# pyannote/pyannote-audio

Measured on AMD Instinct MI355X. Metric: audio-hours/sec (real-time factor) for speaker-diarization-3.1 pipeline, higher is better.
Workload: dtype f32

## Files before the change

### pyannote-audio_amd/csrc/seg_lstm.hip

```cpp
#include "common.h"

namespace pa {

constexpr int GB = 128;
constexpr int GK = 32;
constexpr int GLD = GK + 4;

template <int ACT, int OUT_MODE>
__global__ __launch_bounds__(256) void k_gemm_tn(const float* __restrict__ A, int lda,
                                                  const float* __restrict__ W, int ldw,
                                                  const float* __restrict__ bias,
                                                  const float* __restrict__ Res,
                                                  float* __restrict__ C, long ldc, int M, int N, int K,
                                                  int nm, int nn, int inner, long sAo, long sAi, long sWo,
                                                  long sWi, long sCo, long sCi, int gHW, int gWo, int gH, int gW) {
  if (gridDim.y > 1) {
    const int zo = blockIdx.y / inner, zi = blockIdx.y % inner;
    A += zo * sAo + zi * sAi;
    W += zo * sWo + zi * sWi;
    C += zo * sCo + zi * sCi;
    if (Res != nullptr) Res += zo * sCo + zi * sCi;
  }
  __shared__ __attribute__((aligned(16))) float As[GB * GLD];
  __shared__ __attribute__((aligned(16))) float Ws[GB * GLD];
  int mt, nt;
  const int bid = blockIdx.x;
  if (nn == 8) {
    nt = (bid >> 3) & 7;
    mt = (bid & 7) + 8 * (bid >> 6);
  } else {
    nt = bid % nn;
    mt = bid / nn;
  }
  if (mt >= nm) return;
  const int m0 = mt * GB, n0 = nt * GB;
  const int tid = threadIdx.x, lane = tid & 63, wv = tid >> 6;
  const int wm = wv >> 1, wn = wv & 1;
  const int lr = tid >> 3, lc = (tid & 7) * 4;

  float4 ra[4], rw[4];
  const float* ap[4];
  const float* wp[4];
#pragma unroll
  for (int i = 0; i < 4; ++i) {
    const int ar = m0 + lr + 32 * i, wr = n0 + lr + 32 * i;
    long arow = ar;
    if (gHW > 0) {
      const int b = ar / gHW, rem = ar - b * gHW, y = rem / gWo, x = rem - y * gWo;
      arow = ((long)b * gH + 2 * y) * gW + 2 * x;
    }
    ap[i] = ar < M ? A + arow * lda + lc : nullptr;
    wp[i] = wr < N ? W + (long)wr * ldw + lc : nullptr;
  }
  auto gload = [&](int k0) {
#pragma unroll
    for (int i = 0; i < 4; ++i) {
      ra[i] = ap[i] != nullptr ? *reinterpret_cast<const float4*>(ap[i] + k0) : make_float4(0.f, 0.f, 0.f, 0.f);
      rw[i] = wp[i] != nullptr ? *reinterpret_cast<const float4*>(wp[i] + k0) : make_float4(0.f, 0.f, 0.f, 0.f);
    }
  };
  auto lstore = [&]() {
#pragma unroll
    for (int i = 0; i < 4; ++i) {
      *reinterpret_cast<float4*>(As + (lr + 32 * i) * GLD + lc) = ra[i];
      *reinterpret_cast<float4*>(Ws + (lr + 32 * i) * GLD + lc) = rw[i];
    }
  };

  f32x16 acc[2][2];
#pragma unroll
  for (int i = 0; i < 2; ++i)
#pragma unroll
    for (int j = 0; j < 2; ++j)
#pragma unroll
      for (int r = 0; r < 16; ++r) acc[i][j][r] = 0.f;

  const int fi = lane & 31, kh = lane >> 5;
  gload(0);
  for (int k0 = 0; k0 < K; k0 += GK) {
    __syncthreads();
    lstore();
    __syncthreads();
    if (k0 + GK < K) gload(k0 + GK);
#pragma unroll
    for (int r4 = 0; r4 < 4; ++r4) {
      float4 af[2], wf[2];
#pragma unroll
      for (int i = 0; i < 2; ++i) {
        af[i] = *reinterpret_cast<const float4*>(As + (64 * wm + 32 * i + fi) * GLD + kh * 16 + 4 * r4);
        wf[i] = *reinterpret_cast<const float4*>(Ws + (64 * wn + 32 * i + fi) * GLD + kh * 16 + 4 * r4);
      }
#pragma unroll
      for (int i = 0; i < 2; ++i)
#pragma unroll
        for (int j = 0; j < 2; ++j) {
          acc[i][j] = MFMA32(af[i].x, wf[j].x, acc[i][j]);
          acc[i][j] = MFMA32(af[i].y, wf[j].y, acc[i][j]);
          acc[i][j] = MFMA32(af[i].z, wf[j].z, acc[i][j]);
          acc[i][j] = MFMA32(af[i].w, wf[j].w, acc[i][j]);
        }
    }
  }

#pragma unroll
  for (int i = 0; i < 2; ++i)
#pragma unroll
    for (int j = 0; j < 2; ++j) {
      const int n = n0 + 64 * wn + 32 * j + fi;
      const float bv = (bias != nullptr && n < N) ? bias[n] : 0.f;
#pragma unroll
      for (int q = 0; q < 4; ++q) {
        const int m = m0 + 64 * wm + 32 * i + 8 * q + 4 * kh;
        float v[4];
#pragma unroll
        for (int e = 0; e < 4; ++e) {
          v[e] = acc[i][j][4 * q + e] + bv;
          if (OUT_MODE == 0 && Res != nullptr && n < N && m + e < M) v[e] += Res[(long)(m + e) * ldc + n];
          if (ACT == 1) v[e] = leaky_relu(v[e]);
          if (ACT == 2) v[e] = fmaxf(v[e], 0.f);
          if (ACT == 3) v[e] = gelu_erf(v[e]);
        }
        if (n < N) {
          if (OUT_MODE == 0) {
#pragma unroll
            for (int e = 0; e < 4; ++e)
              if (m + e < M) C[(long)(m + e) * ldc + n] = v[e];
          } else {
            if (m < M)
              *reinterpret_cast<float4*>(C + ((long)(m >> 4) * N + n) * 16 + (m & 15)) =
                  make_float4(v[0], v[1], v[2], v[3]);
          }
        }
      }
    }
}

constexpr int LSTM_HS = 162;

__device__ __forceinline__ float sigmoidf_(float x) {
  return __builtin_amdgcn_rcpf(1.0f + __builtin_amdgcn_exp2f(-1.4426950408889634f * x));
}
__device__ __forceinline__ float tanhf_(float x) {
  const float xc = fminf(fmaxf(x, -15.f), 15.f);
  return 2.0f * __builtin_amdgcn_rcpf(1.0f + __builtin_amdgcn_exp2f(-2.8853900817779268f * xc)) - 1.0f;
}

__global__ __launch_bounds__(256, 1) void k_lstm_rec(const float* __restrict__ xproj,
                                                      const float* __restrict__ whh_p,
                                                      float* __restrict__ out, int T) {
  __shared__ float hs[2 * 16 * LSTM_HS];
  const int tile = blockIdx.x, dir = blockIdx.y;
  const int tid = threadIdx.x, lane = tid & 63, w = tid >> 6;
  const int n = lane & 15, g = lane >> 4;

  float wr[8][32];
  {
    const float* wp = whh_p + (long)((dir * 4 + w) * 8 * 32) * 64 + lane;
#pragma unroll
    for (int q8 = 0; q8 < 8; ++q8)
#pragma unroll
      for (int kt = 0; kt < 32; ++kt) wr[q8][kt] = wp[(q8 * 32 + kt) * 64];
  }
  for (int i = tid; i < 2 * 16 * LSTM_HS; i += 256) hs[i] = 0.f;
  float c[2][4];
#pragma unroll
  for (int s = 0; s < 2; ++s)
#pragma unroll
    for (int r = 0; r < 4; ++r) c[s][r] = 0.f;
  __syncthreads();

  const float* xbase = xproj + ((long)tile * T * 1024 + dir * 512 + w * 128 + n) * 16 + 4 * g;
  float* obase = out + ((long)tile * T * 16 + 4 * g) * 256 + dir * 128 + 32 * w + n;

  f32x4 xin[8];
  {
    const int t = dir ? T - 1 : 0;
#pragma unroll
    for (int q8 = 0; q8 < 8; ++q8)
      xin[q8] = *reinterpret_cast<const f32x4*>(xbase + ((long)t * 1024 + q8 * 16) * 16);
  }
  int cur = 0;
#pragma unroll 1
  for (int step = 0; step < T; ++step) {
    const int t = dir ? T - 1 - step : step;
    f32x4 acc[8];
#pragma unroll
    for (int q8 = 0; q8 < 8; ++q8) acc[q8] = xin[q8];
    if (step + 1 < T) {
      const int tn = dir ? t - 1 : t + 1;
#pragma unroll
      for (int q8 = 0; q8 < 8; ++q8)
        xin[q8] = *reinterpret_cast<const f32x4*>(xbase + ((long)tn * 1024 + q8 * 16) * 16);
    }
    const float* hp = hs + (cur * 16 + n) * LSTM_HS + g * 33;
    float a[32];
#pragma unroll
    for (int kt = 0; kt < 32; ++kt) a[kt] = hp[kt];
#pragma unroll
    for (int kt = 0; kt < 32; ++kt)
#pragma unroll
      for (int q8 = 0; q8 < 8; ++q8) acc[q8] = MFMA16(a[kt], wr[q8][kt], acc[q8]);

    float* hn = hs + ((cur ^ 1) * 16 + 4 * g) * LSTM_HS + w * 33 + n;
    float* op = obase + (long)t * 16 * 256;
#pragma unroll
    for (int s = 0; s < 2; ++s)
#pragma unroll
      for (int r = 0; r < 4; ++r) {
        const float ig = sigmoidf_(acc[0 + s][r]);
        const float fg = sigmoidf_(acc[2 + s][r]);
        const float gg = tanhf_(acc[4 + s][r]);
        const float og = sigmoidf_(acc[6 + s][r]);
        const float cn = fg * c[s][r] + ig * gg;
        c[s][r] = cn;
        const float h = og * tanhf_(cn);
        hn[r * LSTM_HS + 16 * s] = h;
        op[r * 256 + 16 * s] = h;
      }
    __syncthreads();
    cur ^= 1;
  }
}

constexpr int LSTMG_MT = 2;
constexpr int LSTMG_MAXU = 8;

__global__ __launch_bounds__(256) void k_lstm_rec_gen(const float* __restrict__ xproj,
                                                      const float* __restrict__ whh_g,
                                                      float* __restrict__ out, int T, int H, int ntiles,
                                                      int ndir, int hstride) {
  extern __shared__ float hsg[];
  constexpr int MT = LSTMG_MT;
  const int tile0 = blockIdx.x * MT, dir = blockIdx.y;
  const int tid = threadIdx.x, lane = tid & 63, w = tid >> 6;
  const int n = lane & 15, g = lane >> 4;
  const int U = H >> 4, K4 = H >> 4;
  const long NG = (long)ndir * 4 * H;
  const int ldo = ndir * H;
  for (int i = tid; i < MT * 2 * 16 * hstride; i += 256) hsg[i] = 0.f;
  f32x4 c[LSTMG_MAXU][MT];
#pragma unroll
  for (int ui = 0; ui < LSTMG_MAXU; ++ui)
#pragma unroll
    for (int mt = 0; mt < MT; ++mt) c[ui][mt] = f32x4{0.f, 0.f, 0.f, 0.f};
  __syncthreads();
  int tl[MT];
  bool live[MT];
#pragma unroll
  for (int mt = 0; mt < MT; ++mt) {
    live[mt] = tile0 + mt < ntiles;
    tl[mt] = live[mt] ? tile0 + mt : ntiles - 1;
  }
  int cur = 0;
#pragma unroll 1
  for (int step = 0; step < T; ++step) {
    const int t = dir ? T - 1 - step : step;
#pragma unroll
    for (int ui = 0; ui < LSTMG_MAXU; ++ui) {
      const int u = w + 4 * ui;
      if (u >= U) break;
      f32x4 xin[MT][4], acc[MT][4];
#pragma unroll
      for (int mt = 0; mt < MT; ++mt)
#pragma unroll
        for (int q = 0; q < 4; ++q) {
          xin[mt][q] = *reinterpret_cast<const f32x4*>(
              xproj + (((long)tl[mt] * T + t) * NG + (long)dir * 4 * H + (4 * u + q) * 16 + n) * 16 + 4 * g);
          acc[mt][q] = f32x4{0.f, 0.f, 0.f, 0.f};
        }
      const f32x4* wp = reinterpret_cast<const f32x4*>(whh_g) + ((long)(dir * U + u) * 4 * K4) * 64 + lane;
      const float* hp0 = hsg + (cur * 16 + n) * hstride + g;
#pragma unroll 2
      for (int k4 = 0; k4 < K4; ++k4) {
        f32x4 b[4];
#pragma unroll
        for (int q = 0; q < 4; ++q) b[q] = wp[(long)(q * K4 + k4) * 64];
#pragma unroll
        for (int j = 0; j < 4; ++j) {
#pragma unroll
          for (int mt = 0; mt < MT; ++mt) {
            const float a = hp0[mt * 2 * 16 * hstride + 16 * k4 + 4 * j];
#pragma unroll
            for (int q = 0; q < 4; ++q) acc[mt][q] = MFMA16(a, b[q][j], acc[mt][q]);
          }
        }
      }
#pragma unroll
      for (int mt = 0; mt < MT; ++mt) {
        float* hn = hsg + ((mt * 2 + (cur ^ 1)) * 16 + 4 * g) * hstride + 16 * u + n;
        float* op = out + (((long)tl[mt] * T + t) * 16 + 4 * g) * ldo + dir * H + 16 * u + n;
#pragma unroll
        for (int r = 0; r < 4; ++r) {
          const float ig = sigmoidf_(acc[mt][0][r] + xin[mt][0][r]);
          const float fg = sigmoidf_(acc[mt][1][r] + xin[mt][1][r]);
          const float gg = tanhf_(acc[mt][2][r] + xin[mt][2][r]);
          const float og = sigmoidf_(acc[mt][3][r] + xin[mt][3][r]);
          const float cn = fg * c[ui][mt][r] + ig * gg;
          c[ui][mt][r] = cn;
          const float h = og * tanhf_(cn);
          hn[r * hstride] = h;
          if (live[mt]) op[(long)r * ldo] = h;
        }
      }
    }
    __syncthreads();
    cur ^= 1;
  }
}

constexpr int CLS_MAXC = 16;

__global__ __launch_bounds__(256) void k_classifier(const float* __restrict__ X, int ldx, int K, int M,
                                                     int T, int B, const float* __restrict__ cw,
                                                     const float* __restrict__ cb, int NC,
                                                     const unsigned char* __restrict__ mapping, int S,
                                                     float* __restrict__ logp,
                                                     unsigned char* __restrict__ ml) {
  extern __shared__ float wsh[];
  for (int i = threadIdx.x; i < NC * K; i += 256) wsh[i] = cw[i];
  for (int i = threadIdx.x; i < NC; i += 256) wsh[NC * K + i] = cb[i];
  __syncthreads();
  const long m = (long)blockIdx.x * 256 + threadIdx.x;
  if (m >= M) return;
  const int b16 = (int)(m & 15);
  const long tt = m >> 4;
  const int t = (int)(tt % T), tile = (int)(tt / T);
  const int b = tile * 16 + b16;
  if (b >= B) return;
  float z[CLS_MAXC];
#pragma unroll
  for (int cidx = 0; cidx < CLS_MAXC; ++cidx) z[cidx] = cidx < NC ? wsh[NC * K + cidx] : 0.f;
  const float* x = X + m * ldx;
  for (int k = 0; k < K; k += 4) {
    const float4 xv = *reinterpret_cast<const float4*>(x + k);
#pragma unroll
    for (int cidx = 0; cidx < CLS_MAXC; ++cidx)
      if (cidx < NC) {
        const float* wrow = wsh + cidx * K + k;
        z[cidx] = fmaf(xv.x, wrow[0], z[cidx]);
        z[cidx] = fmaf(xv.y, wrow[1], z[cidx]);
        z[cidx] = fmaf(xv.z, wrow[2], z[cidx]);
        z[cidx] = fmaf(xv.w, wrow[3], z[cidx]);
      }
  }
  const long o = (long)b * T + t;
  if (mapping == nullptr) {
    if (logp != nullptr)
      for (int cidx = 0; cidx < NC; ++cidx) logp[o * NC + cidx] = 1.f / (1.f + expf(-z[cidx]));
    return;
  }
  float mx = z[0];
  int am = 0;
#pragma unroll
  for (int cidx = 1; cidx < CLS_MAXC; ++cidx)
    if (cidx < NC && z[cidx] > mx) {
      mx = z[cidx];
      am = cidx;
    }
  float se = 0.f;
#pragma unroll
  for (int cidx = 0; cidx < CLS_MAXC; ++cidx)
    if (cidx < NC) se += expf(z[cidx] - mx);
  const float lse = mx + logf(se);
  if (logp != nullptr)
    for (int cidx = 0; cidx < NC; ++cidx) logp[o * NC + cidx] = z[cidx] - lse;
  if (ml != nullptr)
    for (int s = 0; s < S; ++s) ml[o * S + s] = mapping[am * S + s];
}

}

extern "C" {

int pa_gemm_tn_ex(const float* A, int lda, const float* W, int ldw, const float* bias, const float* Res,
                  float* C, long ldc, int M, int N, int K, int act, int out_mode, void* stream);

int pa_gemm_tn(const float* A, int lda, const float* W, int ldw, const float* bias, float* C, long ldc,
               int M, int N, int K, int act, int out_mode, void* stream) {
  return pa_gemm_tn_ex(A, lda, W, ldw, bias, nullptr, C, ldc, M, N, K, act, out_mode, stream);
}

int pa_gemm_tn_batched(const float* A, int lda, long sAo, long sAi, const float* W, int ldw, long sWo, long sWi,
                       const float* bias, float* C, long ldc, long sCo, long sCi, int M, int N, int K,
                       int outer, int inner, int act, void* stream);

static int gemm_tn_launch(const float* A, int lda, const float* W, int ldw, const float* bias, const float* Res,
                          float* C, long ldc, int M, int N, int K, int act, int out_mode, int gHW, int gWo, int gH,
                          int gW, void* stream);

int pa_gemm_tn_ex(const float* A, int lda, const float* W, int ldw, const float* bias, const float* Res,
                  float* C, long ldc, int M, int N, int K, int act, int out_mode, void* stream) {
  return gemm_tn_launch(A, lda, W, ldw, bias, Res, C, ldc, M, N, K, act, out_mode, 0, 0, 0, 0, stream);
}

int pa_gemm_tn_s2(const float* X, int B, int H, int W, int cin, const float* Wt, int ldw, const float* bias, float* C,
                  long ldc, int N, void* stream) {
  const int Ho = (H - 1) / 2 + 1, Wo = (W - 1) / 2 + 1;
  if (B <= 0) return 0;
  return gemm_tn_launch(X, cin, Wt, ldw, bias, nullptr, C, ldc, B * Ho * Wo, N, cin, 0, 0, Ho * Wo, Wo, H, W, stream);
}

static int gemm_tn_launch(const float* A, int lda, const float* W, int ldw, const float* bias, const float* Res,
                          float* C, long ldc, int M, int N, int K, int act, int out_mode, int gHW, int gWo, int gH,
                          int gW, void* stream) {
  if (M <= 0 || N <= 0) return 0;
  PA_REQUIRE(Res == nullptr || out_mode == 0, "pa_gemm_tn_ex: a residual needs out_mode 0");
  PA_REQUIRE(K % pa::GK == 0 && lda % 4 == 0 && ldw % 4 == 0,
             "pa_gemm_tn: K (%d) must be a multiple of 32 and lda/ldw multiples of 4", K);
  PA_REQUIRE(out_mode == 0 || (M % 16 == 0), "pa_gemm_tn: out_mode 1 needs M %% 16 == 0");
  const int nm = pa::cdiv(M, pa::GB), nn = pa::cdiv(N, pa::GB);
  const int grid = nn == 8 ? pa::cdiv(nm, 8) * 64 : nm * nn;
  hipStream_t st = (hipStream_t)stream;
  pa::ProfScope prof("k_gemm_tn", stream, 2.0 * M * N * K, 4.0 * ((double)M * K + (double)N * K + (double)M * N));
#define PA_GEMM(ACT, OM)                                                                          \
  hipLaunchKernelGGL((pa::k_gemm_tn<ACT, OM>), dim3(grid), dim3(256), 0, st, A, lda, W, ldw, bias, \
                     Res, C, ldc, M, N, K, nm, nn, 1, 0L, 0L, 0L, 0L, 0L, 0L, gHW, gWo, gH, gW)
  if (act == 0 && out_mode == 0) PA_GEMM(0, 0);
  else if (act == 1 && out_mode == 0) PA_GEMM(1, 0);
  else if (act == 2 && out_mode == 0) PA_GEMM(2, 0);
  else if (act == 3 && out_mode == 0) PA_GEMM(3, 0);
  else if (act == 0 && out_mode == 1) PA_GEMM(0, 1);
  else PA_REQUIRE(false, "pa_gemm_tn: unsupported act/out_mode %d/%d", act, out_mode);
#undef PA_GEMM
  PA_CHECK_LAUNCH("pa_gemm_tn");
  return 0;
}

int pa_gemm_tn_batched(const float* A, int lda, long sAo, long sAi, const float* W, int ldw, long sWo, long sWi,
                       const float* bias, float* C, long ldc, long sCo, long sCi, int M, int N, int K,
                       int outer, int inner, int act, void* stream) {
  if (M <= 0 || N <= 0 || outer <= 0 || inner <= 0) return 0;
  PA_REQUIRE(K % pa::GK == 0 && lda % 4 == 0 && ldw % 4 == 0 && sAo % 4 == 0 && sAi % 4 == 0 && sWo % 4 == 0 &&
                 sWi % 4 == 0,
             "pa_gemm_tn_batched: K (%d) must be a multiple of 32 and every stride a multiple of 4", K);
  PA_REQUIRE((long)outer * inner <= 65535, "pa_gemm_tn_batched: at most 65535 products per launch");
  const int nm = pa::cdiv(M, pa::GB), nn = pa::cdiv(N, pa::GB);
  const int grid = nn == 8 ? pa::cdiv(nm, 8) * 64 : nm * nn;
  hipStream_t st = (hipStream_t)stream;
  const double z = (double)outer * inner;
  pa::ProfScope prof("k_gemm_tn", stream, 2.0 * z * M * N * K, 4.0 * z * ((double)M * K + (double)N * K + (double)M * N));
#define PA_GEMMB(ACT)                                                                                          \
  hipLaunchKernelGGL((pa::k_gemm_tn<ACT, 0>), dim3(grid, outer * inner), dim3(256), 0, st, A, lda, W, ldw, bias, \
                     (const float*)nullptr, C, ldc, M, N, K, nm, nn, inner, sAo, sAi, sWo, sWi, sCo, sCi, 0, 0, 0, 0)
  if (act == 0) PA_GEMMB(0);
  else if (act == 3) PA_GEMMB(3);
  else PA_REQUIRE(false, "pa_gemm_tn_batched: unsupported act %d", act);
#undef PA_GEMMB
  PA_CHECK_LAUNCH("pa_gemm_tn_batched");
  return 0;
}

int pa_lstm_rec(const float* xproj, const float* whh_packed, float* out, int ntiles, int ndir, int T,
                void* stream) {
  if (ntiles <= 0 || T <= 0) return 0;
  pa::ProfScope prof("k_lstm_rec", stream, 2.0 * ntiles * 16 * ndir * T * 128 * 512,
                     4.0 * ntiles * 16 * ndir * T * (512 + 128));
  hipLaunchKernelGGL(pa::k_lstm_rec, dim3(ntiles, ndir), dim3(256), 0, (hipStream_t)stream, xproj,
                     whh_packed, out, T);
  PA_CHECK_LAUNCH("pa_lstm_rec");
  return 0;
}

int pa_lstm_rec_h(const float* xproj, const float* whh_packed, float* out, int ntiles, int ndir, int T, int H,
                  void* stream) {
  if (ntiles <= 0 || T <= 0) return 0;
  if (H == 128 && ndir == 2) return pa_lstm_rec(xproj, whh_packed, out, ntiles, ndir, T, stream);
  PA_REQUIRE(H >= 16 && H % 16 == 0 && H <= 64 * pa::LSTMG_MAXU && (ndir == 1 || ndir == 2),
             "pa_lstm_rec_h: hidden size %d must be a multiple of 16 in [16, %d], directions 1 or 2 (got %d)", H,
             64 * pa::LSTMG_MAXU, ndir);
  const int hstride = ((H + 63) / 64) * 64 + 4;
  const size_t lds = sizeof(float) * pa::LSTMG_MT * 2 * 16 * hstride;
  {
    int dev = 0, limit = 0;
    (void)hipGetDevice(&dev);
    (void)hipDeviceGetAttribute(&limit, hipDeviceAttributeMaxSharedMemoryPerBlock, dev);
    PA_REQUIRE(limit <= 0 || lds <= (size_t)limit,
               "pa_lstm_rec_h: hidden size %d needs %zu bytes of LDS per workgroup, this device offers %d", H, lds, limit);
    static size_t granted = 0;
    if (lds > granted) {
      PA_REQUIRE(hipFuncSetAttribute((const void*)pa::k_lstm_rec_gen, hipFuncAttributeMaxDynamicSharedMemorySize,
                                     (int)lds) == hipSuccess,
                 "pa_lstm_rec_h: cannot reserve %zu bytes of dynamic LDS for hidden size %d", lds, H);
      granted = lds;
    }
  }
  pa::ProfScope prof("k_lstm_rec_gen", stream, 2.0 * ntiles * 16 * ndir * T * H * 4.0 * H,
                     4.0 * ntiles * 16 * ndir * T * (4.0 * H + H));
  hipLaunchKernelGGL(pa::k_lstm_rec_gen, dim3(pa::cdiv(ntiles, pa::LSTMG_MT), ndir), dim3(256), lds,
                     (hipStream_t)stream, xproj, whh_packed, out, T, H, ntiles, ndir, hstride);
  PA_CHECK_LAUNCH("pa_lstm_rec_h");
  return 0;
}

int pa_classifier(const float* X, int ldx, int K, int ntiles, int T, int B, const float* cw,
                  const float* cb, int NC, const unsigned char* mapping, int S, float* logp,
                  unsigned char* multilabel, void* stream) {
  PA_REQUIRE(NC <= pa::CLS_MAXC && K % 4 == 0, "pa_classifier: NC <= 16 and K %% 4 == 0 required");
  const long M = (long)ntiles * T * 16;
  if (M <= 0) return 0;
  const size_t lds = (size_t)(NC * K + NC) * sizeof(float);
  pa::ProfScope prof("k_classifier", stream, 2.0 * M * K * NC, 4.0 * M * K + 4.0 * M * NC);
  hipLaunchKernelGGL(pa::k_classifier, dim3(pa::cdiv(M, 256)), dim3(256), lds, (hipStream_t)stream, X,
                     ldx, K, (int)M, T, B, cw, cb, NC, mapping, S, logp, multilabel);
  PA_CHECK_LAUNCH("pa_classifier");
  return 0;
}

}
```

Measured before the change: 1.344.

## Prefetch LSTM input projections into LDS and add opt-in persistent gate GEMM

The LSTM recurrence kernel gains a variant, on by default, that prefetches the next timestep's input projection through buffer_load-to-LDS instructions interleaved with the MFMA chain. It then reads that data from LDS after the gate math, instead of holding the next step's inputs in VGPRs via global loads. This aims to hide global latency on the serial recurrent critical path, at the cost of 64KB of dynamic LDS. A new persistent, tile-queue-driven gate GEMM kernel with direct-to-LDS loads and a blocked output layout is also added, but it is only used when PA_GATE_GEMM is set.

```diff
diff --git a/pyannote-audio_amd/csrc/seg_gemm_gates.hip b/pyannote-audio_amd/csrc/seg_gemm_gates.hip
--- /dev/null
+++ b/pyannote-audio_amd/csrc/seg_gemm_gates.hip
@@ -0,0 +1,310 @@
+#include "common.h"
+
+namespace pa {
+
+constexpr int GG_B = 128;
+constexpr int GG_K = 32;
+constexpr int GG_IMG = GG_B * GG_K * 4;
+constexpr int GG_W_BASE = 2 * GG_IMG;
+constexpr int GG_BIAS_BASE = 4 * GG_IMG;
+constexpr int GG_MAIL = GG_BIAS_BASE + 2048;
+constexpr int GG_LDS = GG_MAIL + 16;
+constexpr int GG_OOB = (int)0x80000000;
+constexpr int GG_PIECES = 8;
+constexpr int GG_TILE_STORES = 16;
+#define GG_STR2(x) #x
+#define GG_STR(x) GG_STR2(x)
+#define GG_TAIL_WAIT_LIT 16
+static_assert(GG_TILE_STORES == GG_TAIL_WAIT_LIT, "the literal of the s_waitcnt string");
+
+typedef __attribute__((address_space(3))) unsigned char* gg_lds_t;
+typedef const volatile f32x4 __attribute__((address_space(3))) * gg_lds_f32x4_ptr;
+typedef const volatile float __attribute__((address_space(3))) * gg_lds_f32_ptr;
+__device__ __forceinline__ f32x4 gg_lds_read128(gg_lds_t p) { return *(gg_lds_f32x4_ptr)p; }
+
+__device__ __forceinline__ void gg_barrier() {
+  asm volatile("s_waitcnt lgkmcnt(0)" ::: "memory");
+  __builtin_amdgcn_s_barrier();
+  asm volatile("" ::: "memory");
+}
+
+template <int IMM>
+__device__ __forceinline__ void gg_piece(unsigned dst, int voff, __amdgpu_buffer_rsrc_t srd, int soff) {
+  asm volatile("s_add_u32 m0, %0, %1\n\ts_nop 0\n\tbuffer_load_dwordx4 %2, %3, %4 offen lds"
+               :: "s"(dst), "i"(IMM), "v"(voff), "s"(srd), "s"(soff)
+               : "memory", "scc");
+}
+struct GgStage {
+  __amdgpu_buffer_rsrc_t asrd, wsrd, bsrd;
+  int soff;
+  unsigned adst, wdst;
+  unsigned bdst;
+  bool with_bias;
+};
+template <int N>
+__device__ __forceinline__ void gg_issue(const GgStage& st, const int (&aoff)[4], const int (&woff)[4]) {
+  if constexpr (N < 4) gg_piece<4096 * N>(st.adst, aoff[N], st.asrd, st.soff);
+  else gg_piece<4096 * (N - 4)>(st.wdst, woff[N - 4], st.wsrd, st.soff);
+}
+__device__ __forceinline__ void gg_issue_n(const int n, const GgStage& st, const int (&aoff)[4], const int (&woff)[4]) {
+  switch (n) {
+#define GG_CASE(I) case I: gg_issue<I>(st, aoff, woff); break;
+    GG_CASE(0) GG_CASE(1) GG_CASE(2) GG_CASE(3) GG_CASE(4) GG_CASE(5) GG_CASE(6) GG_CASE(7)
+#undef GG_CASE
+    default: break;
+  }
+}
+
+__global__ __launch_bounds__(256, 2) void k_gemm_gates(const float* __restrict__ A, int lda,
+                                                       const float* __restrict__ W, int ldw,
+                                                       const float* __restrict__ bias, float* __restrict__ C, int M,
+                                                       int N, int K, int nm, int nn, int* __restrict__ counters) {
+  extern __shared__ __attribute__((aligned(16))) unsigned char smem_gg[];
+  const gg_lds_t lds = (gg_lds_t)smem_gg;
+  const unsigned lds0 = (unsigned)(size_t)lds;
+  int* mail = reinterpret_cast<int*>(smem_gg + GG_MAIL);
+
+  const int tid = threadIdx.x, lane = tid & 63;
+  const int slw = __builtin_amdgcn_readfirstlane(tid >> 6);
+  const int wm = slw >> 1, wn = slw & 1;
+  const int fi = lane & 31, kh = lane >> 5;
+
+  struct Tile {
+    int m0, n0;
+  };
+  auto mt_of = [&](int t) { return ((t >> 3) / nn) * 8 + (t & 7); };
+  auto decode = [&](int t) {
+    Tile q;
+    q.m0 = mt_of(t) * GG_B;
+    q.n0 = ((t >> 3) % nn) * GG_B;
+    return q;
+  };
+  auto resolve = [&](const TileQueue& tqq, int r) {
+    for (;;) {
+      const int t = tq_resolve(tqq, r);
+      if (t < 0 || mt_of(t) < nm) return t;
+      r = tq_claim_own(tqq);
+    }
+  };
+
+  gg_lds_t pa_[4], pw_[4];
+#pragma unroll
+  for (int r4 = 0; r4 < 4; ++r4) {
+    const int slot = ((4 * kh + r4) ^ ((fi >> 1) & 7)) * 16;
+    pa_[r4] = lds + (64 * wm + fi) * 128 + slot;
+    pw_[r4] = lds + GG_W_BASE + (64 * wn + fi) * 128 + slot;
+    asm volatile("" : "+v"(pa_[r4]));
+    asm volatile("" : "+v"(pw_[r4]));
+  }
+  const int drow = 8 * slw + (lane >> 3);
+  const int dslot = (lane & 7) ^ (4 * (slw & 1) + (lane >> 4));
+  int woff[4], aoff[4], arel[4];
+#pragma unroll
+  for (int j = 0; j < 4; ++j) {
+    woff[j] = ((drow + 32 * j) * ldw + 4 * dslot) * 4;
+    arel[j] = ((drow + 32 * j) * lda + 4 * dslot) * 4;
+  }
+  auto tile_offsets = [&](const Tile& q) {
+    const int rows = M - q.m0;
+#pragma unroll
+    for (int j = 0; j < 4; ++j) aoff[j] = drow + 32 * j < rows ? arel[j] : GG_OOB;
+  };
+  const int boff = lane < 32 ? lane * 16 : GG_OOB;
+  auto a_srd = [&](const Tile& q, bool live) {
+    const int rows = M - q.m0 < GG_B ? M - q.m0 : GG_B;
+    return __builtin_amdgcn_make_buffer_rsrc(const_cast<float*>(A + (long)q.m0 * lda), 0,
+                                             live ? ((rows - 1) * lda + K) * 4 : 0, 0x00020000);
+  };
+  auto w_srd = [&](const Tile& q, bool live) {
+    return __builtin_amdgcn_make_buffer_rsrc(const_cast<float*>(W + (long)q.n0 * ldw), 0,
+                                             live ? ((GG_B - 1) * ldw + K) * 4 : 0, 0x00020000);
+  };
+  auto b_srd = [&](const Tile& q, bool live) {
+    return __builtin_amdgcn_make_buffer_rsrc(const_cast<float*>(bias != nullptr ? bias + q.n0 : W), 0,
+                                             bias != nullptr && live ? GG_B * 4 : 0, 0x00020000);
+  };
+
+  const int per_xcd = ((nm + 7) >> 3) * nn;
+  const TileQueue tq{counters, (int)(blockIdx.x & 7), per_xcd};
+  if (tid == 0) mail[0] = resolve(tq, tq_claim_own(tq));
+  __syncthreads();
+  const int t0 = __builtin_amdgcn_readfirstlane(mail[0]);
+  if (t0 < 0) {
+    if (tid == 0) tq_done(tq, gridDim.x);
+    return;
+  }
+  Tile cur = decode(t0), nxt = cur;
+  __amdgpu_buffer_rsrc_t acur = a_srd(cur, true), wcur = w_srd(cur, true);
+  tile_offsets(cur);
+  {
+    GgStage st;
+    st.asrd = acur;
+    st.wsrd = wcur;
+    st.soff = 0;
+    st.adst = lds0 + 1024 * slw;
+    st.wdst = lds0 + GG_W_BASE + 1024 * slw;
+#pragma unroll
+    for (int n = 0; n < GG_PIECES; ++n) gg_issue_n(n, st, aoff, woff);
+    if (slw == 0) gg_piece<0>(lds0 + GG_BIAS_BASE, boff, b_srd(cur, true), 0);
+  }
+  int claim = 0;
+  if (tid == 0) claim = tq_claim_own(tq);
+  const int nst = K / GG_K;
+  int buf = 0, par = 0, tn = -1;
+  bool first_tile = true;
+
+  for (;;) {
+    f32x16 acc[2][2];
+#pragma unroll
+    for (int i = 0; i < 2; ++i)
+#pragma unroll
+      for (int j = 0; j < 2; ++j)
+#pragma unroll
+        for (int r = 0; r < 16; ++r) acc[i][j][r] = 0.f;
+    for (int s = 0; s < nst; ++s) {
+      const bool last = s == nst - 1;
+      if (s == 0 && !first_tile) asm volatile("s_waitcnt vmcnt(" GG_STR(GG_TAIL_WAIT_LIT) ")" ::: "memory");
+      else asm volatile("s_waitcnt vmcnt(0)" ::: "memory");
+      if (last && tid == 0) mail[par ^ 1] = resolve(tq, claim);
+      gg_barrier();
+      GgStage st;
+      auto setup = [&]() {
+        st.asrd = acur;
+        st.wsrd = wcur;
+        st.bsrd = wcur;
+        if (last) {
+          tn = __builtin_amdgcn_readfirstlane(mail[par ^ 1]);
+          if (tn >= 0) {
+            nxt = decode(tn);
+            tile_offsets(nxt);
+          }
+          st.asrd = a_srd(nxt, tn >= 0);
+          st.wsrd = w_srd(nxt, tn >= 0);
+          st.bsrd = b_srd(nxt, tn >= 0);
+        }
+        st.soff = last ? 0 : (s + 1) * GG_K * 4;
+        st.adst = lds0 + (buf ^ 1) * GG_IMG + 1024 * slw;
+        st.wdst = lds0 + GG_W_BASE + (buf ^ 1) * GG_IMG + 1024 * slw;
+        st.bdst = lds0 + GG_BIAS_BASE + (par ^ 1) * 1024;
+        st.with_bias = last && slw == 0;
+      };
+
+      {
+        f32x4 fa[2][2], fw[2][2];
+        auto rd = [&](const int r4, const int n, const int p) {
+          if (n == 0) fa[p][0] = gg_lds_read128(pa_[r4]);
+          else if (n == 1) fw[p][0] = gg_lds_read128(pw_[r4]);
+          else if (n == 2) fw[p][1] = gg_lds_read128(pw_[r4] + 4096);
+          else fa[p][1] = gg_lds_read128(pa_[r4] + 4096);
+        };
+#pragma unroll
+        for (int n = 0; n < 4; ++n) rd(0, n, 0);
+        __builtin_amdgcn_sched_barrier(0);
+        setup();
+        __builtin_amdgcn_sched_barrier(0);
+#pragma unroll
+        for (int r4 = 0; r4 < 4; ++r4) {
+          const int p = r4 & 1;
+#pragma unroll
+          for (int m = 0; m < 16; ++m) {
+            const int e = m >> 2, i = (m >> 1) & 1, j = m & 1;
+            acc[i][j] = MFMA32(fa[p][i][e], fw[p][j][e], acc[i][j]);
+            __builtin_amdgcn_sched_barrier(0);
+            if (r4 + 1 < 4 && m < 4) {
+              rd(r4 + 1, m, p ^ 1);
+              __builtin_amdgcn_sched_barrier(0);
+            }
+            const int idx = 16 * r4 + m;
+            if ((idx & 7) == 5) {
+              gg_issue_n(idx >> 3, st, aoff, woff);
+              __builtin_amdgcn_sched_barrier(0);
+            }
+            if (idx == 62) {
+              if (st.with_bias) gg_piece<0>(st.bdst, boff, st.bsrd, 0);
+              __builtin_amdgcn_sched_barrier(0);
+            }
+          }
+        }
+      }
+      {
+        const int d = buf ? -GG_IMG : GG_IMG;
+#pragma unroll
+        for (int r4 = 0; r4 < 4; ++r4) {
+          pa_[r4] += d;
+          pw_[r4] += d;
+          asm volatile("" : "+v"(pa_[r4]));
+          asm volatile("" : "+v"(pw_[r4]));
+        }
+      }
+      buf ^= 1;
+    }
+    if (tid == 0 && tn >= 0) claim = tq_claim_own(tq);
+    first_tile = false;
+    {
+      const int gv = (M - cur.m0) >> 4;
+      const __amdgpu_buffer_rsrc_t csrd = __builtin_amdgcn_make_buffer_rsrc(
+          C + ((long)(cur.m0 >> 4) * N + cur.n0) * 16, 0, (((gv < 8 ? gv : 8) - 1) * N + GG_B) * 64, 0x00020000);
+      const gg_lds_f32_ptr bl = (gg_lds_f32_ptr)(lds + GG_BIAS_BASE + par * 1024 + (64 * wn + fi) * 4);
+      const float bv[2] = {bl[0], bl[32]};
+      const int lane_base = (64 * wn + (fi & 15)) * 64 + (fi >> 4) * 32 + kh * 16;
+#pragma unroll
+      for (int i = 0; i < 2; ++i)
+#pragma unroll
+        for (int gg = 0; gg < 2; ++gg) {
+          const int gl = 4 * wm + 2 * i + gg;
+          const int voff = gl < gv ? gl * N * 64 + lane_base : GG_OOB;
+#pragma unroll
+          for (int j = 0; j < 2; ++j) {
+            u32x4 x, y;
+#pragma unroll
+            for (int e = 0; e < 4; ++e) {
+              const float lo = acc[i][j][8 * gg + e] + bv[j], hi = acc[i][j][8 * gg + 4 + e] + bv[j];
+              const auto r = __builtin_amdgcn_permlane16_swap(__builtin_bit_cast(unsigned int, lo),
+                                                              __builtin_bit_cast(unsigned int, hi), false, false);
+              x[e] = r[0];
+              y[e] = r[1];
+            }
+            __builtin_amdgcn_raw_buffer_store_b128(x, csrd, voff + j * 2048, 0, 0);
+            __builtin_amdgcn_raw_buffer_store_b128(y, csrd, voff + (j * 2048 + 1024), 0, 0);
+            asm volatile("s_nop 1" ::: "memory");
+            __builtin_amdgcn_sched_barrier(0);
+          }
+        }
+    }
+    if (tn < 0) break;
+    cur = nxt;
+    acur = a_srd(cur, true);
+    wcur = w_srd(cur, true);
+    par ^= 1;
+  }
+  if (tid == 0) tq_done(tq, gridDim.x);
+}
+
+int launch_gemm_gates(const float* A, int lda, const float* W, int ldw, const float* bias, float* C, int M, int N,
+                      int K, hipStream_t st) {
+  constexpr int MAXDEV = 16;
+  static int resident_of[MAXDEV] = {0};
+  int dev = 0;
+  (void)hipGetDevice(&dev);
+  if (dev < 0 || dev >= MAXDEV) dev = 0;
+  if (!resident_of[dev]) {
+    (void)hipFuncSetAttribute((const void*)k_gemm_gates, hipFuncAttributeMaxDynamicSharedMemorySize, GG_LDS);
+    int cus = 256;
+    (void)hipDeviceGetAttribute(&cus, hipDeviceAttributeMultiprocessorCount, dev);
+    resident_of[dev] = 2 * cus;
+  }
+  const int resident = resident_of[dev] & ~7;
+  const int nm = cdiv(M, GG_B), nn = N / GG_B;
+  const long total = (long)nm * nn;
+  const int grid = (int)(total < resident ? total : resident);
+  int* counters = tile_counters();
+  if (counters == nullptr) {
+    set_error("pa_gemm_tn: cannot allocate the tile counters");
+    return 2;
+  }
+  hipLaunchKernelGGL(k_gemm_gates, dim3(grid), dim3(256), GG_LDS, st, A, lda, W, ldw, bias, C, M, N, K, nm, nn,
+                     counters);
+  return 0;
+}
+
+}
diff --git a/pyannote-audio_amd/csrc/seg_lstm.hip b/pyannote-audio_amd/csrc/seg_lstm.hip
--- a/pyannote-audio_amd/csrc/seg_lstm.hip
+++ b/pyannote-audio_amd/csrc/seg_lstm.hip
@@ -145,10 +145,22 @@
   return 2.0f * __builtin_amdgcn_rcpf(1.0f + __builtin_amdgcn_exp2f(-2.8853900817779268f * xc)) - 1.0f;
 }
 
+constexpr int LSTM_XIN_WAVE = 2 * 8 * 1024;
+typedef __attribute__((address_space(3))) unsigned char* lstm_lds_t;
+typedef const volatile f32x4 __attribute__((address_space(3))) * lstm_lds_f32x4_ptr;
+template <int IMM>
+__device__ __forceinline__ void lstm_xin_piece(unsigned dst, int voff, __amdgpu_buffer_rsrc_t srd, int soff) {
+  asm volatile("s_add_u32 m0, %0, %1\n\ts_nop 0\n\tbuffer_load_dwordx4 %2, %3, %4 offen lds"
+               :: "s"(dst), "i"(IMM), "v"(voff), "s"(srd), "s"(soff)
+               : "memory", "scc");
+}
+
+template <bool XLDS>
 __global__ __launch_bounds__(256, 1) void k_lstm_rec(const float* __restrict__ xproj,
                                                       const float* __restrict__ whh_p,
                                                       float* __restrict__ out, int T) {
   __shared__ float hs[2 * 16 * LSTM_HS];
+  extern __shared__ __attribute__((aligned(16))) unsigned char xin_lds[];
   const int tile = blockIdx.x, dir = blockIdx.y;
   const int tid = threadIdx.x, lane = tid & 63, w = tid >> 6;
   const int n = lane & 15, g = lane >> 4;
@@ -172,12 +184,37 @@
   const float* xbase = xproj + ((long)tile * T * 1024 + dir * 512 + w * 128 + n) * 16 + 4 * g;
   float* obase = out + ((long)tile * T * 16 + 4 * g) * 256 + dir * 128 + 32 * w + n;
 
+  const int slw = __builtin_amdgcn_readfirstlane(w);
+  const __amdgpu_buffer_rsrc_t xsrd = __builtin_amdgcn_make_buffer_rsrc(
+      const_cast<float*>(xproj + ((long)tile * T * 1024 + dir * 512 + slw * 128) * 16), 0,
+      XLDS ? (T - 1) * 65536 + 8192 : 0, 0x00020000);
+  const int xvoff = n * 64 + g * 16;
+  const unsigned xdst = (unsigned)(size_t)(lstm_lds_t)xin_lds + slw * LSTM_XIN_WAVE;
+  lstm_lds_t xrd = (lstm_lds_t)xin_lds + slw * LSTM_XIN_WAVE + lane * 16;
+  auto xin_piece = [&](const int P, unsigned dst, __amdgpu_buffer_rsrc_t srd, int soff) {
+    switch (P) {
+#define PA_XIN_CASE(I) case I: lstm_xin_piece<I * 1024>(dst, xvoff, srd, soff + I * 1024); break;
+      PA_XIN_CASE(0) PA_XIN_CASE(1) PA_XIN_CASE(2) PA_XIN_CASE(3) PA_XIN_CASE(4) PA_XIN_CASE(5) PA_XIN_CASE(6)
+      PA_XIN_CASE(7)
+#undef PA_XIN_CASE
+      default: break;
+    }
+  };
+
   f32x4 xin[8];
   {
     const int t = dir ? T - 1 : 0;
-#pragma unroll
-    for (int q8 = 0; q8 < 8; ++q8)
-      xin[q8] = *reinterpret_cast<const f32x4*>(xbase + ((long)t * 1024 + q8 * 16) * 16);
+    if constexpr (XLDS) {
+#pragma unroll
+      for (int P = 0; P < 8; ++P) xin_piece(P, xdst, xsrd, t * 65536);
+      asm volatile("s_waitcnt vmcnt(0)" ::: "memory");
+#pragma unroll
+      for (int q8 = 0; q8 < 8; ++q8) xin[q8] = *(lstm_lds_f32x4_ptr)(xrd + q8 * 1024);
+    } else {
+#pragma unroll
+      for (int q8 = 0; q8 < 8; ++q8)
+        xin[q8] = *reinterpret_cast<const f32x4*>(xbase + ((long)t * 1024 + q8 * 16) * 16);
+    }
   }
   int cur = 0;
 #pragma unroll 1
@@ -186,11 +223,19 @@
     f32x4 acc[8];
 #pragma unroll
     for (int q8 = 0; q8 < 8; ++q8) acc[q8] = xin[q8];
-    if (step + 1 < T) {
-      const int tn = dir ? t - 1 : t + 1;
-#pragma unroll
-      for (int q8 = 0; q8 < 8; ++q8)
-        xin[q8] = *reinterpret_cast<const f32x4*>(xbase + ((long)tn * 1024 + q8 * 16) * 16);
+    const bool more = step + 1 < T;
+    const __amdgpu_buffer_rsrc_t nsrd = __builtin_amdgcn_make_buffer_rsrc(
+        const_cast<float*>(xproj + ((long)tile * T * 1024 + dir * 512 + slw * 128) * 16), 0,
+        XLDS && more ? (T - 1) * 65536 + 8192 : 0, 0x00020000);
+    const unsigned ndst = xdst + (cur ^ 1) * 8192;
+    const int nsoff = more ? (dir ? t - 1 : t + 1) * 65536 : 0;
+    if constexpr (!XLDS) {
+      if (step + 1 < T) {
+        const int tn = dir ? t - 1 : t + 1;
+#pragma unroll
+        for (int q8 = 0; q8 < 8; ++q8)
+          xin[q8] = *reinterpret_cast<const f32x4*>(xbase + ((long)tn * 1024 + q8 * 16) * 16);
+      }
     }
     const float* hp = hs + (cur * 16 + n) * LSTM_HS + g * 33;
     float a[32];
@@ -199,7 +244,16 @@
 #pragma unroll
     for (int kt = 0; kt < 32; ++kt)
 #pragma unroll
-      for (int q8 = 0; q8 < 8; ++q8) acc[q8] = MFMA16(a[kt], wr[q8][kt], acc[q8]);
+      for (int q8 = 0; q8 < 8; ++q8) {
+        acc[q8] = MFMA16(a[kt], wr[q8][kt], acc[q8]);
+        if constexpr (XLDS) {
+          if (q8 == 7 && (kt & 3) == 1) {
+            __builtin_amdgcn_sched_barrier(0);
+            xin_piece(kt >> 2, ndst, nsrd, nsoff);
+            __builtin_amdgcn_sched_barrier(0);
+          }
+        }
+      }
 
     float* hn = hs + ((cur ^ 1) * 16 + 4 * g) * LSTM_HS + w * 33 + n;
     float* op = obase + (long)t * 16 * 256;
@@ -217,6 +271,12 @@
         hn[r * LSTM_HS + 16 * s] = h;
         op[r * 256 + 16 * s] = h;
       }
+    if constexpr (XLDS) {
+      asm volatile("s_waitcnt vmcnt(8)" ::: "memory");
+      xrd += cur ? -8192 : 8192;
+#pragma unroll
+      for (int q8 = 0; q8 < 8; ++q8) xin[q8] = *(lstm_lds_f32x4_ptr)(xrd + q8 * 1024);
+    }
     __syncthreads();
     cur ^= 1;
   }
@@ -368,6 +428,9 @@
     for (int s = 0; s < S; ++s) ml[o * S + s] = mapping[am * S + s];
 }
 
+int launch_gemm_gates(const float* A, int lda, const float* W, int ldw, const float* bias, float* C, int M, int N,
+                      int K, hipStream_t st);
+
 }
 
 extern "C" {
@@ -412,7 +475,17 @@
   const int grid = nn == 8 ? pa::cdiv(nm, 8) * 64 : nm * nn;
   hipStream_t st = (hipStream_t)stream;
   pa::ProfScope prof("k_gemm_tn", stream, 2.0 * M * N * K, 4.0 * ((double)M * K + (double)N * K + (double)M * N));
-#define PA_GEMM(ACT, OM)                                                                          \
+  if (out_mode == 1 && act == 0 && gHW == 0 && N % 128 == 0 && N <= (1 << 20) && lda <= (1 << 20) &&
+      ldw <= (1 << 20)) {
+    const char* e = getenv("PA_GATE_GEMM");
+    if (e != nullptr && atoi(e) != 0) {
+      const int rc = pa::launch_gemm_gates(A, lda, W, ldw, bias, C, M, N, K, st);
+      if (rc != 0) return rc;
+      PA_CHECK_LAUNCH("pa_gemm_tn");
+      return 0;
+    }
+  }
+#define PA_GEMM(ACT, OM)                                                                         \
   hipLaunchKernelGGL((pa::k_gemm_tn<ACT, OM>), dim3(grid), dim3(256), 0, st, A, lda, W, ldw, bias, \
                      Res, C, ldc, M, N, K, nm, nn, 1, 0L, 0L, 0L, 0L, 0L, 0L, gHW, gWo, gH, gW)
   if (act == 0 && out_mode == 0) PA_GEMM(0, 0);
@@ -455,8 +528,22 @@
   if (ntiles <= 0 || T <= 0) return 0;
   pa::ProfScope prof("k_lstm_rec", stream, 2.0 * ntiles * 16 * ndir * T * 128 * 512,
                      4.0 * ntiles * 16 * ndir * T * (512 + 128));
-  hipLaunchKernelGGL(pa::k_lstm_rec, dim3(ntiles, ndir), dim3(256), 0, (hipStream_t)stream, xproj,
-                     whh_packed, out, T);
+  const char* e = getenv("PA_LSTM_XIN_LDS");
+  if ((e == nullptr || atoi(e) != 0) && T <= 32000) {
+    constexpr int lds = 4 * pa::LSTM_XIN_WAVE;
+    static bool granted = false;
+    if (!granted) {
+      PA_REQUIRE(hipFuncSetAttribute((const void*)pa::k_lstm_rec<true>, hipFuncAttributeMaxDynamicSharedMemorySize,
+                                     lds) == hipSuccess,
+                 "pa_lstm_rec: cannot reserve %d bytes of dynamic LDS", lds);
+      granted = true;
+    }
+    hipLaunchKernelGGL(pa::k_lstm_rec<true>, dim3(ntiles, ndir), dim3(256), lds, (hipStream_t)stream, xproj,
+                       whh_packed, out, T);
+  } else {
+    hipLaunchKernelGGL(pa::k_lstm_rec<false>, dim3(ntiles, ndir), dim3(256), 0, (hipStream_t)stream, xproj,
+                       whh_packed, out, T);
+  }
   PA_CHECK_LAUNCH("pa_lstm_rec");
   return 0;
 }
```

Result: no change. 1.348, median of 6 (+0.3%).
